# GetOverMassif/QSP-SLAM

Hardware: AMD Instinct MI355X
Metric: joint-opt iters/sec (BA+SDF) (higher is better)
Workload: dtype f32 as 2 x fp16 per operand (hi + 2^-11 lo'), 3 fp16 products per multiply-add, f32 accumulate (decoder); f64 (bundle adjustment)

## Files before the change

include/qsp_hip.h:

```cpp
#ifndef QSP_HIP_H
#define QSP_HIP_H

#include <stddef.h>
#include <stdint.h>

#ifdef __cplusplus
extern "C" {
#endif

enum {
    QSP_OK = 0,
    QSP_ERR_INVALID = 1,
    QSP_ERR_UNSUPPORTED = 2,
    QSP_ERR_DEVICE = 3,
    QSP_ERR_NO_DEVICE = 4
};

const char* qsp_last_error(void);
int qsp_version(void);
int qsp_device_count(void);


typedef struct {
    int32_t n_layers;
    int32_t code_len;
    int32_t latent_in_layer;
    const int32_t* in_dim;
    const int32_t* out_dim;
    const float* const* weight;
    const float* const* weight_g;
    const float* const* bias;
} qsp_decoder_desc;

typedef struct qsp_decoder qsp_decoder;

int qsp_decoder_create(const qsp_decoder_desc* desc, int device, qsp_decoder** out);
void qsp_decoder_destroy(qsp_decoder* dec);

enum { QSP_DEC_OPT_FORWARD_PRECISION = 1, QSP_DEC_OPT_JACOBIAN_PRECISION = 2, QSP_DEC_OPT_TILE_POINTS = 3,
       QSP_DEC_OPT_RENDER_SCREENING = 4, QSP_DEC_OPT_USE_TANH = 5, QSP_DEC_OPT_RANGE_FALLBACK = 6,
       QSP_DEC_OPT_SCREENING_MIN_SAMPLES = 7, QSP_DEC_OPT_NARROW_TILE = 8, QSP_DEC_OPT_SCREEN_AUDIT = 9,
       QSP_DEC_OPT_DEPTH_STAGING = 10 };
enum { QSP_DEC_CNT_RANGE_FALLBACKS = 1, QSP_DEC_CNT_ARENA_REUSED = 2, QSP_DEC_CNT_ARENA_CREATED = 3, QSP_DEC_CNT_NARROW_TILE = 4,
       QSP_DEC_CNT_SCREEN_FALLBACKS = 5 };
int64_t qsp_decoder_get_counter(qsp_decoder* dec, int32_t counter);
int qsp_decoder_set_option(qsp_decoder* dec, int32_t option, int32_t value);

int qsp_decode_sdf(qsp_decoder* dec, const float* code, const float* xyz, int64_t n, float* sdf_out);

int qsp_decode_sdf_screen(qsp_decoder* dec, const float* code, const float* xyz, int64_t n, float* s1_out);

int qsp_sdf_value_grad(qsp_decoder* dec, const float* code, const float* xyz, int64_t n, float* y, float* grad);

typedef struct {
    float k1, k2, k3, k4;
    float b1, b2;
    float lr;
    float s_damp;
    float cut_off;
    int32_t n_iter;
    int32_t n_depth;
    int32_t code_len;
} qsp_joint_cfg;

typedef struct qsp_refine_batch qsp_refine_batch;

int qsp_refine_batch_create(qsp_decoder* dec, const qsp_joint_cfg* cfg, int32_t n_obj,
                            const float* const* pts, const int32_t* n_pts,
                            const float* const* rays, const int32_t* n_rays,
                            const float* const* depth, const int32_t* n_fg,
                            int32_t n_hyp, const int32_t* hyp_obj, qsp_refine_batch** out);
void qsp_refine_batch_destroy(qsp_refine_batch* b);

int qsp_refine_batch_set_state(qsp_refine_batch* b, const float* t_cam_obj, const float* code);

int qsp_refine_batch_run(qsp_refine_batch* b, int32_t n_iter);

int qsp_refine_batch_get(qsp_refine_batch* b, float* t_cam_obj_out, float* code_out, float* loss_out,
                         uint8_t* is_good_out);

int qsp_refine_batch_trace(qsp_refine_batch* b, float* H, float* rhs, float* dx, int32_t* n_valid,
                           int32_t* n_render, float* loss_terms);
int qsp_refine_batch_trace_rot(qsp_refine_batch* b, float* rot4);

int qsp_refine_batch_rows(qsp_refine_batch* b, int enable, int32_t hyp, float* rows_sdf, float* rows_render);

typedef struct {
    float ms_total;
    float ms_mlp_jtj;
    float ms_mlp_fwd;
    float ms_other;
    int32_t n_launch_jtj, n_launch_fwd;
    int64_t pts_jtj;
    int64_t pts_fwd;
    int64_t tiles_jtj, tiles_fwd;
    int64_t pts_band;
    int32_t range_fallbacks;
    int32_t screen_fallbacks;
    float screen_max_diff;
    int32_t screen_audit_failures;
    int64_t pts_audit;
} qsp_refine_profile;
int qsp_refine_batch_profile(qsp_refine_batch* b, int enable, qsp_refine_profile* out);
// ... 490 lines not shown
```

qsp_slam_amd/_lib.py:

```python
import ctypes as C
import os

import numpy as np

_HERE = os.path.dirname(os.path.abspath(__file__))
LIB_PATH = os.environ.get("QSP_HIP_LIB", os.path.join(_HERE, "libqsp_hip.so"))

QSP_OK, QSP_ERR_INVALID, QSP_ERR_UNSUPPORTED, QSP_ERR_DEVICE, QSP_ERR_NO_DEVICE = 0, 1, 2, 3, 4

c_float_p = C.POINTER(C.c_float)
c_double_p = C.POINTER(C.c_double)
c_int32_p = C.POINTER(C.c_int32)
c_int64_p = C.POINTER(C.c_int64)
c_uint8_p = C.POINTER(C.c_uint8)


class QspError(RuntimeError):
    def __init__(self, code, msg):
        RuntimeError.__init__(self, "qsp_hip error %d: %s" % (code, msg))
        self.code = code


class DecoderDesc(C.Structure):
    _fields_ = [("n_layers", C.c_int32), ("code_len", C.c_int32), ("latent_in_layer", C.c_int32),
# ... 137 lines not shown
class FuseOut(C.Structure):
    _fields_ = [("best_idx", c_int32_p), ("best_dist", c_int32_p), ("reason", c_int32_p), ("level", c_int32_p)]


class SearchProjIn(C.Structure):
    _fields_ = [("mode", C.c_int32), ("frame", C.POINTER(OrbFrame)), ("K", C.c_float * 5), ("Ow", C.c_float * 3), ("mb", C.c_float),
                ("u_right", c_float_p), ("slot_blocked", c_uint8_p), ("kp_angle", c_float_p),
                ("th", C.c_float), ("nn_ratio", C.c_float), ("view_cos_limit", C.c_float), ("check_orientation", C.c_int32), ("mono", C.c_int32),
                ("last_Rcw", C.c_float * 9), ("last_tcw", C.c_float * 3), ("n_src", C.c_int32),
                ("src_valid", c_uint8_p), ("src_blocks", c_uint8_p), ("Xw", c_float_p), ("desc", c_uint8_p), ("normal", c_float_p),
                ("dist_min_inv", c_float_p), ("dist_max_inv", c_float_p), ("dist_max", c_float_p), ("src_octave", c_int32_p), ("src_angle", c_float_p)]


class SearchProjOut(C.Structure):
    _fields_ = [("choice", c_int32_p), ("dist", c_int32_p), ("slot_src", c_int32_p), ("in_view", c_uint8_p), ("proj_x", c_float_p),
                ("proj_y", c_float_p), ("proj_xr", c_float_p), ("level", c_int32_p), ("view_cos", c_float_p), ("reason", c_int32_p),
                ("dist2", c_int32_p), ("level_best", c_int32_p), ("level2", c_int32_p), ("bin", c_int32_p), ("n_matches", C.c_int32),
                ("hist", C.c_int32 * 30), ("ind", C.c_int32 * 3), ("n_rounds", C.c_int32)]


class SearchProjKfIn(C.Structure):
    _fields_ = [("mode", C.c_int32), ("frame", C.POINTER(OrbFrame)), ("K", C.c_float * 4), ("Ow", C.c_float * 3),
                ("slot_blocked", c_uint8_p), ("kp_angle", c_float_p), ("th", C.c_float), ("orb_dist", C.c_int32),
                ("check_orientation", C.c_int32), ("n_src", C.c_int32), ("src_valid", c_uint8_p), ("Xw", c_float_p), ("desc", c_uint8_p),
                ("dist_min_inv", c_float_p), ("dist_max_inv", c_float_p), ("dist_max", c_float_p), ("normal", c_float_p),
                ("src_angle", c_float_p)]


class SearchProjKfOut(C.Structure):
    _fields_ = [("choice", c_int32_p), ("dist", c_int32_p), ("slot_src", c_int32_p), ("reason", c_int32_p), ("level", c_int32_p),
                ("proj_x", c_float_p), ("proj_y", c_float_p), ("bin", c_int32_p), ("n_matches", C.c_int32),
                ("hist", C.c_int32 * 30), ("ind", C.c_int32 * 3), ("n_rounds", C.c_int32)]


class TriangulateFrame(C.Structure):
    _fields_ = [("n", C.c_int32), ("Rcw", C.c_float * 9), ("tcw", C.c_float * 3), ("Ow", C.c_float * 3),
                ("fx", C.c_float), ("fy", C.c_float), ("cx", C.c_float), ("cy", C.c_float), ("invfx", C.c_float), ("invfy", C.c_float),
                ("mb", C.c_float), ("mbf", C.c_float), ("xy_un", c_float_p), ("xy", c_float_p), ("u_right", c_float_p), ("depth", c_float_p),
                ("sigma2", c_float_p), ("scale", c_float_p)]


class TriangulateGeom(C.Structure):
    _fields_ = [("n_cand", C.c_int32), ("kf1", C.POINTER(TriangulateFrame)), ("kf2", C.POINTER(TriangulateFrame)), ("ratio_factor", C.c_float)]


class TriangulateOut(C.Structure):
    _fields_ = [("accept", c_uint8_p), ("first", c_uint8_p), ("x3D", c_float_p), ("n_new", c_int32_p), ("reason", c_int32_p), ("path", c_int32_p),
                ("cos_rays", c_float_p), ("z", c_float_p), ("err2", c_float_p), ("ratio_dist", c_float_p)]


SYMBOLS = [
    "qsp_last_error", "qsp_version", "qsp_device_count",
    "qsp_decoder_create", "qsp_decoder_destroy", "qsp_decoder_set_option", "qsp_decoder_get_counter", "qsp_decode_sdf",
    "qsp_decode_sdf_screen", "qsp_sdf_value_grad",
    "qsp_refine_batch_create", "qsp_refine_batch_destroy", "qsp_refine_batch_set_state", "qsp_refine_batch_run",
    "qsp_refine_batch_get", "qsp_refine_batch_trace", "qsp_refine_batch_trace_rot", "qsp_refine_batch_profile", "qsp_refine_batch_rows",
    "qsp_reconstruct_objects", "qsp_estimate_pose", "qsp_refine_detections",
    "qsp_decoder_group_create", "qsp_decoder_group_destroy", "qsp_refine_batch_create_group", "qsp_reconstruct_objects_group",
    "qsp_estimate_pose_group", "qsp_refine_detections_group",
    "qsp_mesh_extractor_create", "qsp_mesh_extractor_destroy", "qsp_mesh_extract", "qsp_mesh_from_volume", "qsp_mesh_fetch", "qsp_mesh_fetch_f64", "qsp_mesh_extractor_set_method",
    "qsp_mesh_extract_batch", "qsp_mesh_from_volumes", "qsp_mesh_fetch_batch", "qsp_mesh_extractor_set_batch_limit",
    "qsp_mesh_extractor_create_group", "qsp_mesh_extract_batch_group",
    "qsp_mc_tables",
    "qsp_pose_optimizer_create", "qsp_pose_optimizer_destroy", "qsp_pose_optimize", "qsp_ellipsoid_fit_planes", "qsp_ellipsoid_fit_prior",
    "qsp_sim3_optimize_batch", "qsp_sim3_ransac_batch", "qsp_search_by_sim3_batch", "qsp_search_by_bow_batch", "qsp_search_for_triangulation_batch", "qsp_fuse_batch", "qsp_search_by_projection", "qsp_search_by_projection_kf", "qsp_triangulate_batch", "qsp_create_new_map_points_batch", "qsp_essential_graph_optimize", "qsp_essential_graph_stages", "qsp_object_gates",
    "qsp_ba_create", "qsp_ba_destroy", "qsp_ba_set_levels", "qsp_ba_optimize", "qsp_ba_local_joint",
    "qsp_ba_set_state", "qsp_ba_get_state", "qsp_ba_get_edges", "qsp_ba_get_index", "qsp_ba_profile", "qsp_ba_set_shard", "qsp_ba_set_deterministic",
    "qsp_ba_set_shard_rccl", "qsp_ba_set_option", "qsp_ba_release_caches", "qsp_comm_unique_id", "qsp_comm_create", "qsp_comm_adopt", "qsp_comm_destroy", "qsp_comm_nccl", "qsp_comm_stub_counts",
    "qsp_comm_rank", "qsp_comm_world", "qsp_comm_allreduce_f64", "qsp_comm_allgather_f32",
]


def lib():
    global _lib
    if _lib is not None:
        return _lib
    if not os.path.isfile(LIB_PATH):
        raise QspError(QSP_ERR_NO_DEVICE, "libqsp_hip.so not built (%s); run qsp_slam_amd/csrc/build.sh -- there is "
                       "no CPU fallback" % LIB_PATH)
    L = C.CDLL(LIB_PATH)
    L.qsp_last_error.restype = C.c_char_p
    L.qsp_version.restype = C.c_int
    L.qsp_device_count.restype = C.c_int
    vp = C.c_void_p
    L.qsp_decoder_create.argtypes = [C.POINTER(DecoderDesc), C.c_int, C.POINTER(vp)]
    L.qsp_decoder_destroy.argtypes = [vp]
    L.qsp_decoder_set_option.argtypes = [vp, C.c_int32, C.c_int32]
    L.qsp_decoder_get_counter.argtypes = [vp, C.c_int32]
    L.qsp_decoder_get_counter.restype = C.c_int64
    L.qsp_decoder_destroy.restype = None
    L.qsp_decode_sdf.argtypes = [vp, c_float_p, c_float_p, C.c_int64, c_float_p]
    L.qsp_decode_sdf_screen.argtypes = [vp, c_float_p, c_float_p, C.c_int64, c_float_p]
    L.qsp_sdf_value_grad.argtypes = [vp, c_float_p, c_float_p, C.c_int64, c_float_p, c_float_p]
    pp_f = C.POINTER(c_float_p)
    L.qsp_refine_batch_create.argtypes = [vp, C.POINTER(JointCfg), C.c_int32, pp_f, c_int32_p, pp_f, c_int32_p, pp_f,
                                          c_int32_p, C.c_int32, c_int32_p, C.POINTER(vp)]
    L.qsp_refine_batch_destroy.argtypes = [vp]
    L.qsp_refine_batch_destroy.restype = None
    L.qsp_refine_batch_set_state.argtypes = [vp, c_float_p, c_float_p]
    L.qsp_refine_batch_run.argtypes = [vp, C.c_int32]
    L.qsp_refine_batch_get.argtypes = [vp, c_float_p, c_float_p, c_float_p, c_uint8_p]
    L.qsp_refine_batch_trace.argtypes = [vp, c_float_p, c_float_p, c_float_p, c_int32_p, c_int32_p, c_float_p]
    L.qsp_refine_batch_trace_rot.argtypes = [vp, c_float_p]
    L.qsp_refine_batch_profile.argtypes = [vp, C.c_int, C.POINTER(RefineProfile)]
    L.qsp_refine_batch_rows.argtypes = [vp, C.c_int, C.c_int32, c_float_p, c_float_p]
    L.qsp_reconstruct_objects.argtypes = [vp, C.POINTER(JointCfg), C.c_int32, pp_f, c_int32_p, pp_f, c_int32_p, pp_f,
                                          c_int32_p, C.c_int32, c_int32_p, c_float_p, c_float_p, c_float_p, c_float_p,
                                          c_float_p, c_uint8_p]
    L.qsp_estimate_pose.argtypes = [vp, C.c_int32, c_float_p, c_float_p, pp_f, c_int32_p, c_float_p, C.c_int32,
                                    c_float_p]
    L.qsp_refine_detections.argtypes = [vp, C.POINTER(JointCfg), C.POINTER(Detections), C.POINTER(DetectionResults)]
    L.qsp_decoder_group_create.argtypes = [C.POINTER(vp), C.c_int32, C.POINTER(vp)]
    L.qsp_decoder_group_destroy.argtypes = [vp]
    L.qsp_decoder_group_destroy.restype = None
    L.qsp_refine_batch_create_group.argtypes = [vp, C.POINTER(JointCfg), C.c_int32, pp_f, c_int32_p, pp_f, c_int32_p, pp_f,
                                                c_int32_p, c_int32_p, C.c_int32, c_int32_p, C.POINTER(vp)]
    L.qsp_reconstruct_objects_group.argtypes = [vp, C.POINTER(JointCfg), C.c_int32, pp_f, c_int32_p, pp_f, c_int32_p, pp_f,
                                                c_int32_p, c_int32_p, C.c_int32, c_int32_p, c_float_p, c_float_p, c_float_p,
                                                c_float_p, c_float_p, c_uint8_p]
    L.qsp_estimate_pose_group.argtypes = [vp, C.c_int32, c_float_p, c_float_p, pp_f, c_int32_p, c_float_p, c_int32_p, C.c_int32,
                                          c_float_p]
    L.qsp_refine_detections_group.argtypes = [vp, C.POINTER(JointCfg), C.POINTER(Detections), c_int32_p, C.POINTER(DetectionResults)]
    L.qsp_mesh_extractor_create.argtypes = [vp, C.c_int32, c_float_p, C.POINTER(vp)]
    L.qsp_mesh_extractor_destroy.argtypes = [vp]
    L.qsp_mesh_extractor_destroy.restype = None
    L.qsp_mesh_extract.argtypes = [vp, c_float_p, c_int64_p, c_int64_p]
    L.qsp_mesh_from_volume.argtypes = [vp, c_float_p, c_int64_p, c_int64_p]
    L.qsp_mesh_fetch.argtypes = [vp, c_float_p, c_int32_p, c_float_p]
    L.qsp_mesh_fetch_f64.argtypes = [vp, C.POINTER(C.c_double)]
    L.qsp_mesh_extractor_set_method.argtypes = [vp, C.c_int32]
    L.qsp_mesh_extract_batch.argtypes = [vp, C.c_int32, c_float_p, c_int64_p, c_int64_p]
    L.qsp_mesh_from_volumes.argtypes = [vp, C.c_int32, c_float_p, c_int64_p, c_int64_p]
    L.qsp_mesh_fetch_batch.argtypes = [vp, c_float_p, C.POINTER(C.c_double), c_int32_p, c_float_p]
    L.qsp_mesh_extractor_set_batch_limit.argtypes = [vp, C.c_int32]
    L.qsp_mesh_extractor_create_group.argtypes = [vp, C.c_int32, c_float_p, C.POINTER(vp)]
    L.qsp_mesh_extract_batch_group.argtypes = [vp, C.c_int32, c_float_p, c_int32_p, c_int64_p, c_int64_p]
    L.qsp_mc_tables.argtypes = [C.POINTER(C.c_int8), C.POINTER(C.c_int8)]
    L.qsp_pose_optimizer_create.argtypes = [C.c_int, C.c_int32, C.POINTER(vp)]
    L.qsp_pose_optimizer_destroy.argtypes = [vp]
    L.qsp_pose_optimizer_destroy.restype = None
    L.qsp_pose_optimize.argtypes = [vp, C.c_int32, c_double_p, c_double_p, c_double_p, c_double_p, c_double_p, c_uint8_p,
                                    c_double_p, c_uint8_p, c_int32_p, C.POINTER(PoseTrace)]
    L.qsp_ellipsoid_fit_planes.argtypes = [C.c_int, C.c_int32, c_double_p, c_int32_p, c_double_p, C.c_int32, C.c_int32,
                                           c_double_p, c_double_p, c_int32_p, c_double_p]
    L.qsp_ellipsoid_fit_prior.argtypes = [C.c_int, C.c_int32, c_double_p, c_int32_p, c_double_p, c_int32_p, c_double_p, c_double_p,
# ... 87 lines not shown
```

qsp_slam_amd/csrc/sdf_mlp.hpp:

```cpp
#pragma once
#include <hip/hip_runtime.h>
#include <stdint.h>

namespace qsp {

typedef float f32x16 __attribute__((ext_vector_type(16)));

#ifndef QSP_EXP_VARIANT
#define QSP_EXP_VARIANT 0
#endif
#if (QSP_EXP_VARIANT & 16)
__device__ unsigned long long qsp_dbg_ts[96];
__device__ unsigned long long qsp_dbg_rt[96];
__device__ int qsp_dbg_n;
#define QSP_TS()                                                                        \
    if (blockIdx.x == 0 && blockIdx.y == 0 && threadIdx.x == 0 && ts_n < 96) {          \
        qsp_dbg_rt[ts_n] = __builtin_amdgcn_s_memrealtime();                            \
        qsp_dbg_ts[ts_n++] = __builtin_readcyclecounter();                              \
        qsp_dbg_n = ts_n;                                                               \
    }
#define QSP_TSK(i)                                                                      \
    if (blockIdx.x == 0 && threadIdx.x == 0 && tsk_first) {                             \
        qsp_dbg_rt[80 + (i)] = __builtin_amdgcn_s_memrealtime();                        \
        qsp_dbg_ts[80 + (i)] = __builtin_readcyclecounter();                            \
    }
#else
#define QSP_TS()
#define QSP_TSK(i)
#endif

constexpr int TILE_P = 64;
constexpr int HID = 512;
constexpr int CODE_LEN = 64;
constexpr int NIN = CODE_LEN + 3;
constexpr int SKIP_COL = HID - NIN;
constexpr int K4 = SKIP_COL + 3;
constexpr int KG4 = K4 / 8;
constexpr int K0_PAD = 96;
constexpr int LDA = HID + 4;
constexpr int LDST = 68;
constexpr int STASH_SHIFT = 1;
static_assert((SKIP_COL - STASH_SHIFT) % 4 == 0 && STASH_SHIFT + NIN <= LDST, "stash row: aligned quads of units 444.., 67 inputs");
constexpr int LDJ = 96;
constexpr int NJ = 72;
constexpr int MLP_THREADS = 512;
constexpr int HT_TILES = 6;

struct MlpParams {
    const float4* wf[8];
    const float4* wb[8];
    const float* bias[8];
    const float* w8;
    float b8;
    const float* w0c;
    const float* w4c;
    const float4* w0x;
    const float4* wf3[8];
    const float4* wb3[8];
    const float4* wfh[8];
    const float4* wbh[8];
    const float4* wbh4s;
    int* range_flag;
    int use_tanh;
    int narrow;
    uint8_t skip[8];
    uint8_t ks_in[8];
    uint8_t ks_out[8];
    uint8_t ncb_in[8];
    uint8_t ncb_out[8];
};

__device__ __forceinline__ float mlp_output(float t, int use_tanh, float& dy) {
    float y = tanhf(t);
    dy = 1.f - y * y;
    if (use_tanh) {
        const float y2 = tanhf(y);
        dy = (1.f - y2 * y2) * dy;
        y = y2;
    }
    return y;
}

struct __attribute__((aligned(16))) MlpSmem {
    float act[TILE_P * LDA];
    float stash[TILE_P * LDST];
    float xin[TILE_P * 4];
    float code[CODE_LEN];
    float c0[HID];
    float c4[HID];
    float y[TILE_P];
    float red[8 * TILE_P];
    float rscale[TILE_P];
    float rres[TILE_P];
    float w8[HID];
    float dy[TILE_P];
};

template <bool AG>
__device__ __forceinline__ f32x16 mfma32t(float a, float b, f32x16 c) {
    if (AG) {
        asm("v_mfma_f32_32x32x2_f32 %0, %1, %2, %0" : "+a"(c) : "v"(a), "v"(b));
        return c;
    }
    return __builtin_amdgcn_mfma_f32_32x32x2f32(a, b, c, 0, 0, 0);
}
template <bool AG>
__device__ __forceinline__ void mfma_acc_settle(f32x16& c0, f32x16& c1, f32x16& c2, f32x16& c3) {
    if (AG) asm volatile("s_nop 15\n\ts_nop 7" : "+a"(c0), "+a"(c1), "+a"(c2), "+a"(c3));
}
template <bool AG>
__device__ __forceinline__ void mfma_acc_settle(f32x16& c0) {
    if (AG) asm volatile("s_nop 15\n\ts_nop 7" : "+a"(c0));
// ... 1314 lines not shown
#pragma unroll
                    for (int q = 0; q < 4; ++q)
                        if (k0 + q < NIN) s.stash[p * LDST + STASH_SHIFT + k0 + q] = sk[r][g][q];
                }
            }
        }
        QSP_BWDH(4, KSH, QSP_WBH(3))
        QSP_BWDH(3, KS4, QSP_WBH(2))
        QSP_BWDH(2, KSH, QSP_WBH(1))
        QSP_BWDH(1, KSH, QSP_WBH(1))
#undef QSP_BWDH
        {
            constexpr int BPT = HID / NT;
            float bnext[7 * BPT];
#pragma unroll
            for (int l = 1; l < 8; ++l)
#pragma unroll
                for (int i = 0; i < BPT; ++i) bnext[BPT * (l - 1) + i] = P.bias[l][tid + i * NT];
            __builtin_amdgcn_sched_barrier(0);
            f32x4 gl[NR][4];
            gemm_side_h2<PF, NR, NW, NARROW>(img, P.wbh[0], wave, lane, gl, NARROW ? (int)P.ks_out[0] : KSH);
            const int c0 = side_c0<NR, NW>(wave);
            __syncthreads();
#pragma unroll
            for (int r = 0; r < NR; ++r) {
                if (r >= side_count<NR, NW>(wave)) break;
                const int p = 32 * side_row<NR, NW>(wave, r) + (lane & 31);
#pragma unroll
                for (int g = 0; g < 4; ++g) {
                    const int k0 = 32 * c0 + 8 * g + 4 * h;
                    if (k0 < NIN) {
                        const float* st = s.stash + p * LDST + STASH_SHIFT + k0;
                        f32x4 v;
#pragma unroll
                        for (int q = 0; q < 4; ++q) v[q] = gl[r][g][q] + (k0 + q < NIN ? st[q] : 0.f);
                        *reinterpret_cast<f32x4*>(s.act + p * LDG + k0) = v;
                    }
                }
            }
            __syncthreads();
#pragma unroll
            for (int l = 1; l < 8; ++l)
#pragma unroll
                for (int i = 0; i < BPT; ++i) bias_sh[(l - 1) * HID + tid + i * NT] = bnext[BPT * (l - 1) + i];
        }
    }
#undef QSP_WH
#undef QSP_WBH
#undef QSP_PIN_ACC
}

constexpr int H1_ROWS = 128;
constexpr int LDH1 = HID + 8;
struct __attribute__((aligned(16))) MlpSmemH1 {
    _Float16 img[H1_ROWS * LDH1 + 64];
    float bias[7 * HID];
    float c0[HID];
    float c4[HID];
    float w8[HID];
    float xin[H1_ROWS * 4];
    float y[H1_ROWS];
    float red[4 * H1_ROWS];
};

template <int PF, int NCB>
struct WRingH1 {
    f32x4 q[PF][NCB];
};
template <int PF, int NCB>
__device__ __forceinline__ void ringh1_prime(WRingH1<PF, NCB>& R, const float4* __restrict__ w_, int cs, int lane) {
    gbytes w = (gbytes)w_;
    const uint32_t voff = 16u * lane;
#pragma unroll
    for (int d = 0; d < PF; ++d)
#pragma unroll
        for (int c = 0; c < NCB; ++c) R.q[d][c] = ldw(w + ((size_t)c * cs + (d * 2) * 64) * 16, voff);
}

template <int KS, int PF, int NCB, int NR>
__device__ __forceinline__ void gemm_h1(const _Float16* __restrict__ img, const float4* __restrict__ w_, int cs,
                                        const float4* __restrict__ nw_, int ncs, WRingH1<PF, NCB>& R, f32x16 (&acc)[NR][NCB], int lane) {
    static_assert(KS % PF == 0 && KS >= 2 * PF && PF % 2 == 0 && NR % NCB == 0, "shape");
    constexpr int RPC = NR / NCB;
    gbytes w = (gbytes)w_;
    gbytes nw = (gbytes)nw_;
    uint32_t voff = 16u * lane;
    int b_idx = (lane & 31) * LDH1 + (lane >> 5) * 8;
    asm volatile("" : "+v"(voff), "+v"(b_idx));
    __builtin_amdgcn_s_waitcnt(0x0F70);
    const _Float16* b_row = img + b_idx;
    f16x8 bh[2][NR];
#pragma unroll
    for (int r = 0; r < NR; ++r) bh[0][r] = *reinterpret_cast<const f16x8*>(b_row + r * 32 * LDH1);
#pragma nounroll
    for (int ks = 0; ks < KS; ks += PF) {
        const bool more = ks + PF < KS;
        gbytes fb = more ? w + (size_t)(ks + PF) * 2 * 64 * 16 : nw;
        const size_t fcs = (size_t)(more ? cs : ncs) * 16;
#pragma unroll
        for (int d = 0; d < PF; ++d) {
            const _Float16* nb = b_row + 16 * (ks + d + 1);
#pragma unroll
            for (int c = 0; c < NCB; ++c) {
                const f16x8 wh = as_f16x8(R.q[d][c]);
#pragma unroll
                for (int r = 0; r < NR; ++r) acc[r][c] = __builtin_amdgcn_mfma_f32_32x32x16_f16(wh, bh[d & 1][r], acc[r][c], 0, 0, 0);
                __builtin_amdgcn_sched_barrier(0);
#pragma unroll
                for (int rr = 0; rr < RPC; ++rr)
                    bh[(d & 1) ^ 1][c * RPC + rr] = *reinterpret_cast<const f16x8*>(nb + (c * RPC + rr) * 32 * LDH1);
                if (c > 0) R.q[d][c - 1] = ldw(fb + (c - 1) * fcs + (size_t)(d * 2) * 64 * 16, voff);
                __builtin_amdgcn_sched_barrier(0);
            }
            R.q[d][NCB - 1] = ldw(fb + (NCB - 1) * fcs + (size_t)(d * 2) * 64 * 16, voff);
            __builtin_amdgcn_sched_barrier(0);
        }
    }
}

__device__ __forceinline__ void h1_store4(_Float16* img, int row, int u0, f32x4 v, float& amax) {
    amax = fmaxf(fmaxf(amax, fabsf(v[0])), fmaxf(fabsf(v[1]), fmaxf(fabsf(v[2]), fabsf(v[3]))));
    asm volatile("" : "+v"(amax));
    f16x4 hi;
#pragma unroll
    for (int q = 0; q < 4; ++q) hi[q] = (_Float16)v[q];
    *reinterpret_cast<f16x4*>(img + row * LDH1 + u0) = hi;
}

template <int PF, int NW = 4>
__device__ __forceinline__ void mlp_tile_h1(MlpSmemH1& s, const MlpParams* __restrict__ Pm, float& amax) {
    constexpr int NR = 4, NCB = 16 / NW;
    int tid = threadIdx.x;
    asm volatile("" : "+v"(tid));
    const int wave = __builtin_amdgcn_readfirstlane(tid >> 6);
    const int lane = tid & 63;
    const int h = lane >> 5;
    int oz;
    asm volatile("s_mov_b32 %0, 0" : "=s"(oz));
    const MlpParams& P = Pm[oz];
    f32x16 acc[NR][NCB];
    _Float16* img = s.img;
    if (tid < H1_ROWS) {
        const f32x4 x = lds4(s.xin + 4 * tid);
        f16x8 hi, z;
#pragma unroll
        for (int j = 0; j < 8; ++j) { hi[j] = (_Float16)0.f; z[j] = (_Float16)0.f; }
#pragma unroll
        for (int j = 0; j < 3; ++j) hi[j] = (_Float16)x[j];
        amax = fmaxf(amax, fmaxf(fabsf(x[0]), fmaxf(fabsf(x[1]), fabsf(x[2]))));
        _Float16* d = img + tid * LDH1;
        *reinterpret_cast<f16x8*>(d) = hi;
        *reinterpret_cast<f16x8*>(d + 8) = z;
    }
    const int cb0 = NCB * wave;
    constexpr int KSH = HID / 16, KS4 = K4 / 16, CS = KSH * 2 * 64, CS4 = KS4 * 2 * 64;
#define QSP_WH(L, KS_) (P.wfh[L] + (size_t)(cb0 * (KS_) * 2) * 64)
    WRingH1<PF, NCB> ring;
    ringh1_prime(ring, QSP_WH(1, KSH), CS, lane);
    __syncthreads();
#define QSP_FWD1(L, BIASPTR, GEMM_STMT)                                                                                  \
    _Pragma("unroll") for (int c_ = 0; c_ < NCB; ++c_) _Pragma("unroll") for (int g_ = 0; g_ < 4; ++g_) {                \
        const f32x4 bv_ = lds4((BIASPTR) + 32 * NCB * wave + 32 * c_ + 8 * g_ + 4 * h);                                  \
        _Pragma("unroll") for (int r_ = 0; r_ < NR; ++r_) _Pragma("unroll") for (int q_ = 0; q_ < 4; ++q_)               \
            acc[r_][c_][4 * g_ + q_] = bv_[q_];                                                                        \
        __builtin_amdgcn_sched_barrier(0);                                                                               \
    }                                                                                                                    \
    GEMM_STMT;                                                                                                           \
     \
     \
    _Pragma("unroll") for (int r_ = 0; r_ < NR; ++r_) _Pragma("unroll") for (int c_ = 0; c_ < NCB; ++c_)                 \
        asm volatile("" : "+a"(acc[r_][c_]));                                                                          \
    __syncthreads();                                                                                                     \
    _Pragma("unroll") for (int c_ = 0; c_ < NCB; ++c_) _Pragma("unroll") for (int g_ = 0; g_ < 4; ++g_) {                \
        const int u0_ = 32 * NCB * wave + 32 * c_ + 8 * g_ + 4 * h;                                                      \
        _Pragma("unroll") for (int r_ = 0; r_ < NR; ++r_) {                                                              \
            f32x4 v_;                                                                                                    \
            _Pragma("unroll") for (int q_ = 0; q_ < 4; ++q_) {                                                           \
                const float x_ = acc[r_][c_][4 * g_ + q_];                                                             \
                v_[q_] = x_ > 0.f ? x_ : 0.f;                                                                            \
            }                                                                                                            \
            h1_store4(img, 32 * r_ + (lane & 31), u0_, v_, amax);                                                        \
        }                                                                                                                \
        __builtin_amdgcn_sched_barrier(0);                                                                               \
    }                                                                                                                    \
    __syncthreads();
#define QSP_GEMM1(L, KS_, NXW, NKS) gemm_h1<KS_, PF, NCB, NR>(img, QSP_WH(L, KS_), (KS_) * 2 * 64, NXW, (NKS) * 2 * 64, ring, acc, lane)
    {
        gbytes w = (gbytes)QSP_WH(0, 1);
        const uint32_t voff = 16u * lane;
        const _Float16* b_row = img + (lane & 31) * LDH1 + (lane >> 5) * 8;
        QSP_FWD1(0, s.c0, {
            f16x8 bh0[NR];
            _Pragma("unroll") for (int r = 0; r < NR; ++r) bh0[r] = *reinterpret_cast<const f16x8*>(b_row + r * 32 * LDH1);
            _Pragma("unroll") for (int c = 0; c < NCB; ++c) {
                const f16x8 wh = as_f16x8(ldw(w + (size_t)(c * 2) * 64 * 16, voff));
                _Pragma("unroll") for (int r = 0; r < NR; ++r)
                    acc[r][c] = __builtin_amdgcn_mfma_f32_32x32x16_f16(wh, bh0[r], acc[r][c], 0, 0, 0);
            }
        })
    }
    QSP_FWD1(1, s.bias + 0 * HID, QSP_GEMM1(1, KSH, QSP_WH(2, KSH), KSH))
    QSP_FWD1(2, s.bias + 1 * HID, QSP_GEMM1(2, KSH, QSP_WH(3, KSH), KSH))
    QSP_FWD1(3, s.bias + 2 * HID, QSP_GEMM1(3, KSH, QSP_WH(4, KS4), KS4))
    if (tid < H1_ROWS) {
#pragma unroll
        for (int ci = 0; ci < 3; ++ci) {
            const float x = s.xin[tid * 4 + ci];
            img[tid * LDH1 + SKIP_COL + ci] = (_Float16)x;
        }
    }
    __syncthreads();
    QSP_FWD1(4, s.c4, QSP_GEMM1(4, KS4, QSP_WH(5, KSH), KSH))
    QSP_FWD1(5, s.bias + 4 * HID, QSP_GEMM1(5, KSH, QSP_WH(6, KSH), KSH))
    QSP_FWD1(6, s.bias + 5 * HID, QSP_GEMM1(6, KSH, QSP_WH(7, KSH), KSH))
    QSP_FWD1(7, s.bias + 6 * HID, QSP_GEMM1(7, KSH, QSP_WH(1, KSH), KSH))
#undef QSP_FWD1
#undef QSP_GEMM1
#undef QSP_WH
    if (NW == 4 || wave < 4) {
        const float* w = s.w8 + 128 * wave;
#pragma unroll
        for (int rr = 0; rr < 2; ++rr) {
            const _Float16* a = img + (lane + 64 * rr) * LDH1 + 128 * wave;
            float pa[4] = {0.f, 0.f, 0.f, 0.f};
#pragma unroll
            for (int g = 0; g < 16; ++g) {
                const f16x8 hi = *reinterpret_cast<const f16x8*>(a + 8 * g);
                const f32x4 w0 = lds4(w + 8 * g), w1 = lds4(w + 8 * g + 4);
#pragma unroll
                for (int j = 0; j < 8; ++j) pa[j & 3] = fmaf((float)hi[j], j < 4 ? w0[j] : w1[j - 4], pa[j & 3]);
            }
            s.red[wave * H1_ROWS + lane + 64 * rr] = (pa[0] + pa[1]) + (pa[2] + pa[3]);
        }
    }
    __syncthreads();
    if (tid < H1_ROWS) {
        float t = P.b8;
#pragma unroll
        for (int q = 0; q < 4; ++q) t += s.red[q * H1_ROWS + tid];
        float dy_;
        s.y[tid] = mlp_output(t, P.use_tanh, dy_);
    }
    __syncthreads();
}

}
```

qsp_slam_amd/csrc/sdf_refine.hip:

```cpp
#include <hip/hip_runtime.h>
#include <math.h>
#include <stdint.h>
#include <stdio.h>
#include <stdlib.h>
#include <string.h>

#include <algorithm>
#include <limits>
#include <string>
#include <mutex>
#include <vector>

#include "../../include/qsp_hip.h"
#include "common.hpp"
#include "sdf_mlp.hpp"

#include "sdf_kernels.hpp"

#ifndef QSP_JTJ_WAVES_DEFAULT
#define QSP_JTJ_WAVES_DEFAULT 8
#endif
#ifndef QSP_SCREEN_WAVES_DEFAULT
#define QSP_SCREEN_WAVES_DEFAULT 4
#endif
// ... 147 lines not shown
    const int in_dim[9] = {NIN, HID, HID, HID, HID, HID, HID, HID, HID};
    const int out_dim[9] = {HID, HID, HID, SKIP_COL, HID, HID, HID, HID, 1};
    auto even4 = [](int v, int cap) { v = std::max(4, (v + 1) & ~1); return std::min(v, cap); };
    double macs = 0, full = 0;
    for (int l = 0; l < 8; ++l) {
        const int in = in_dim[l], out = out_dim[l];
        const int n_hidden = (l == 0) ? 0 : (l == 4 ? SKIP_COL : in);
        int w_out = 0, w_in = 0;
        for (int o = 0; o < out; ++o) {
            bool any = B[l][o] != 0.f;
            for (int k = 0; k < in; ++k)
                if (W[l][(size_t)o * in + k] != 0.f) {
                    any = true;
                    if (k < n_hidden) w_in = std::max(w_in, k + 1);
                }
            if (any) w_out = o + 1;
        }
        const bool skip = src[l] < 0;
        d->P.skip[l] = skip ? 1 : 0;
        const int ks_cap = (l == 4) ? K4 / 16 : HID / 16;
        int ks_in = even4((w_in + 15) / 16, ks_cap);
        if (l == 4 && ks_in >= K4 / 16 - 1) ks_in = K4 / 16;
        d->P.ks_in[l] = (uint8_t)ks_in;
        d->P.ks_out[l] = (uint8_t)even4((w_out + 15) / 16, HID / 16);
        d->P.ncb_in[l] = (uint8_t)std::max(1, (w_in + 31) / 32);
        d->P.ncb_out[l] = (uint8_t)std::max(1, (w_out + 31) / 32);
        full += (double)in * out;
        if (!skip) macs += (double)(l == 0 ? in : 16 * ks_in + (l == 4 ? NIN : 0)) * (32.0 * d->P.ncb_out[l]);
    }
    d->narrow_capable = macs < 0.5 * full;
    d->P.narrow = d->narrow_capable ? 1 : 0;
}

static inline uint16_t bf16_rne(float x) {
    uint32_t u;
    memcpy(&u, &x, 4);
    if ((u & 0x7fffffffu) > 0x7f800000u) return (uint16_t)((u >> 16) | 0x40);
    return (uint16_t)((u + 0x7fffu + ((u >> 16) & 1u)) >> 16);
}
static inline float bf16_f32(uint16_t b) {
    const uint32_t u = (uint32_t)b << 16;
    float x;
    memcpy(&x, &u, 4);
    return x;
}
static inline void bf16_split3(float v, uint16_t& hi, uint16_t& mid, uint16_t& lo) {
    hi = bf16_rne(v);
    const float r1 = v - bf16_f32(hi);
    mid = bf16_rne(r1);
    const float r2 = r1 - bf16_f32(mid);
    lo = bf16_rne(r2);
}

static int pack_weights(qsp_decoder* d, const qsp_decoder_desc* desc) {
    if (desc->n_layers < 1 || desc->n_layers > 64) return qsp_fail(QSP_ERR_UNSUPPORTED, "decoder family: layer count");
    std::vector<std::vector<float>> Wsrc(desc->n_layers);
    for (int l = 0; l < desc->n_layers; ++l) {
        const int in = desc->in_dim[l], out = desc->out_dim[l];
        if (in < 1 || out < 1 || in > 4096 || out > 4096 || !desc->weight[l] || !desc->bias[l])
            return qsp_fail(QSP_ERR_UNSUPPORTED, "decoder family: layer dims");
        Wsrc[l].assign((size_t)out * in, 0.f);
        const float* v = desc->weight[l];
        const float* g = (desc->weight_g && desc->weight_g[l]) ? desc->weight_g[l] : nullptr;
        for (int o = 0; o < out; ++o) {
            float sc = 1.f;
            if (g) {
                float ss = 0.f;
                for (int k = 0; k < in; ++k) ss += v[(size_t)o * in + k] * v[(size_t)o * in + k];
                sc = g[o] / sqrtf(ss);
            }
            for (int k = 0; k < in; ++k) Wsrc[l][(size_t)o * in + k] = v[(size_t)o * in + k] * sc;
        }
        d->mac_per_point += (double)in * out;
    }
    std::vector<std::vector<float>> W, Bias;
    std::vector<int> slot_src;
    {
        const int rc = embed_family(desc, Wsrc, W, Bias, slot_src);
        if (rc) return rc;
    }
    d->code_len = desc->code_len;
    equalize_gains(W, Bias);
    narrow_tables(d, W, Bias, slot_src);
    const int in_dim[9] = {NIN, HID, HID, HID, HID, HID, HID, HID, HID};
    const int out_dim[9] = {HID, HID, HID, SKIP_COL, HID, HID, HID, HID, 1};
    auto upload = [&](const std::vector<float>& h, const void** dst) -> int {
        void* p = nullptr;
        QSP_HIP(hipMalloc(&p, h.size() * sizeof(float) + 16384));
        d->allocs.push_back(p);
        QSP_HIP(hipMemcpy(p, h.data(), h.size() * sizeof(float), hipMemcpyHostToDevice));
        *dst = p;
        return QSP_OK;
    };
    for (int l = 0; l < 8; ++l) {
        const int in = in_dim[l], out = out_dim[l];
        int rc = QSP_OK;
        if (l == 0) {
            std::vector<float> wc((size_t)HID * CODE_LEN), wx((size_t)(HID / 4) * 3 * 4);
            for (int o = 0; o < HID; ++o)
                for (int k = 0; k < CODE_LEN; ++k) wc[(size_t)k * HID + o] = W[0][(size_t)o * in + k];
            for (int q = 0; q < HID / 4; ++q)
                for (int a = 0; a < 3; ++a)
                    for (int e = 0; e < 4; ++e) wx[((size_t)q * 3 + a) * 4 + e] = W[0][(size_t)(4 * q + e) * in + CODE_LEN + a];
            rc = upload(wc, (const void**)&d->P.w0c);
            if (!rc) rc = upload(wx, (const void**)&d->P.w0x);
            d->P.wf[0] = nullptr;
            d->P.wf3[0] = nullptr;
            if (!rc) {
                std::vector<_Float16> ph((size_t)16 * 2 * 64 * 8, (_Float16)0.f);
                for (int cb = 0; cb < 16; ++cb)
                    for (int lane = 0; lane < 64; ++lane)
                        for (int j = 0; j < 8; ++j) {
                            const int o = 32 * cb + (lane & 31), k = 8 * (lane >> 5) + j;
                            float v = 0.f;
                            if (o < out && k < 3) v = W[0][(size_t)o * in + CODE_LEN + k];
                            if (!(fabsf(v) < 65000.f)) d->fp16_ok = false;
                            const _Float16 hi = (_Float16)v;
                            const size_t base = ((size_t)cb * 2) * 64 * 8 + (size_t)lane * 8 + j;
                            ph[base] = hi;
                            ph[base + 64 * 8] = (_Float16)((v - (float)hi) * 2048.f);
                        }
                void* phd = nullptr;
                QSP_HIP(hipMalloc(&phd, ph.size() * sizeof(_Float16) + 16384));
                d->allocs.push_back(phd);
                QSP_HIP(hipMemcpy(phd, ph.data(), ph.size() * sizeof(_Float16), hipMemcpyHostToDevice));
                d->P.wfh[0] = (const float4*)phd;
            }
        } else {
            const int KG = (l == 4) ? KG4 : HID / 8;
            std::vector<float> pf((size_t)16 * KG * 64 * 4, 0.f);
            for (int cb = 0; cb < 16; ++cb)
                for (int kg = 0; kg < KG; ++kg)
                    for (int lane = 0; lane < 64; ++lane)
                        for (int e = 0; e < 4; ++e) {
                            const int o = 32 * cb + (lane & 31);
                            int k = 8 * kg + 4 * (lane >> 5) + e;
                            if (l == 4 && k >= SKIP_COL) k += CODE_LEN;
                            float v = 0.f;
                            if (o < out && k < in) v = W[l][(size_t)o * in + k];
                            pf[(((size_t)cb * KG + kg) * 64 + lane) * 4 + e] = v;
                        }
            rc = upload(pf, (const void**)&d->P.wf[l]);
            if (!rc) {
                const int KS = KG / 2;
                std::vector<uint16_t> p3((size_t)16 * KS * 3 * 64 * 8, 0);
                for (int cb = 0; cb < 16; ++cb)
                    for (int ks = 0; ks < KS; ++ks)
                        for (int lane = 0; lane < 64; ++lane)
                            for (int j = 0; j < 8; ++j) {
                                const int o = 32 * cb + (lane & 31);
                                int k = 16 * ks + 8 * (lane >> 5) + j;
                                if (l == 4 && k >= SKIP_COL) k += CODE_LEN;
                                float v = 0.f;
                                if (o < out && k < in) v = W[l][(size_t)o * in + k];
                                uint16_t hi, mid, lo;
                                bf16_split3(v, hi, mid, lo);
                                const size_t base = (((size_t)cb * KS + ks) * 3) * 64 * 8 + (size_t)lane * 8 + j;
                                p3[base] = hi;
                                p3[base + 64 * 8] = mid;
                                p3[base + 2 * 64 * 8] = lo;
                            }
                void* p3d = nullptr;
                QSP_HIP(hipMalloc(&p3d, p3.size() * sizeof(uint16_t) + 16384));
                d->allocs.push_back(p3d);
                QSP_HIP(hipMemcpy(p3d, p3.data(), p3.size() * sizeof(uint16_t), hipMemcpyHostToDevice));
                d->P.wf3[l] = (const float4*)p3d;
            }
            if (!rc) {
                const int KS = KG / 2;
                std::vector<_Float16> ph((size_t)16 * KS * 2 * 64 * 8, (_Float16)0.f);
                for (int cb = 0; cb < 16; ++cb)
                    for (int ks = 0; ks < KS; ++ks)
                        for (int lane = 0; lane < 64; ++lane)
                            for (int j = 0; j < 8; ++j) {
                                const int o = 32 * cb + (lane & 31);
                                int k = 16 * ks + 8 * (lane >> 5) + j;
                                if (l == 4 && k >= SKIP_COL) k += CODE_LEN;
                                float v = 0.f;
                                if (o < out && k < in) v = W[l][(size_t)o * in + k];
                                if (!(fabsf(v) < 65000.f)) d->fp16_ok = false;
                                const _Float16 hi = (_Float16)v;
                                const _Float16 lo = (_Float16)((v - (float)hi) * 2048.f);
                                const size_t base = (((size_t)cb * KS + ks) * 2) * 64 * 8 + (size_t)lane * 8 + j;
                                ph[base] = hi;
                                ph[base + 64 * 8] = lo;
                            }
                void* phd = nullptr;
                QSP_HIP(hipMalloc(&phd, ph.size() * sizeof(_Float16) + 16384));
                d->allocs.push_back(phd);
                QSP_HIP(hipMemcpy(phd, ph.data(), ph.size() * sizeof(_Float16), hipMemcpyHostToDevice));
                d->P.wfh[l] = (const float4*)phd;
            }
            if (!rc && l == 4) {
                std::vector<float> wc((size_t)HID * CODE_LEN);
                for (int o = 0; o < HID; ++o)
                    for (int k = 0; k < CODE_LEN; ++k) wc[(size_t)k * HID + o] = W[4][(size_t)o * in + SKIP_COL + k];
                rc = upload(wc, (const void**)&d->P.w4c);
            }
        }
        if (rc) return rc;
        const int NCB = (l == 0) ? 3 : 16;
        const int OG = HID / 8;
        std::vector<float> pb((size_t)NCB * OG * 64 * 4, 0.f);
        for (int cb = 0; cb < NCB; ++cb)
            for (int og = 0; og < OG; ++og)
                for (int lane = 0; lane < 64; ++lane)
                    for (int e = 0; e < 4; ++e) {
                        const int k = 32 * cb + (lane & 31);
                        const int o = 8 * og + 4 * (lane >> 5) + e;
                        float v = 0.f;
                        if (o < out && k < in) v = W[l][(size_t)o * in + k];
                        pb[(((size_t)cb * OG + og) * 64 + lane) * 4 + e] = v;
                    }
        rc = upload(pb, (const void**)&d->P.wb[l]);
        if (rc) return rc;
        {
            const int KS = HID / 16;
            std::vector<uint16_t> p3((size_t)NCB * KS * 3 * 64 * 8, 0);
            for (int cb = 0; cb < NCB; ++cb)
                for (int ks = 0; ks < KS; ++ks)
                    for (int lane = 0; lane < 64; ++lane)
                        for (int j = 0; j < 8; ++j) {
                            const int k = 32 * cb + (lane & 31);
                            const int o = 16 * ks + 8 * (lane >> 5) + j;
                            float v = 0.f;
                            if (o < out && k < in) v = W[l][(size_t)o * in + k];
                            uint16_t hi, mid, lo;
                            bf16_split3(v, hi, mid, lo);
                            const size_t base = (((size_t)cb * KS + ks) * 3) * 64 * 8 + (size_t)lane * 8 + j;
                            p3[base] = hi;
                            p3[base + 64 * 8] = mid;
                            p3[base + 2 * 64 * 8] = lo;
                        }
            void* p3d = nullptr;
            QSP_HIP(hipMalloc(&p3d, p3.size() * sizeof(uint16_t) + 16384));
            d->allocs.push_back(p3d);
            QSP_HIP(hipMemcpy(p3d, p3.data(), p3.size() * sizeof(uint16_t), hipMemcpyHostToDevice));
            d->P.wb3[l] = (const float4*)p3d;
        }
        {
            const int KS = HID / 16;
            std::vector<_Float16> ph((size_t)NCB * KS * 2 * 64 * 8, (_Float16)0.f);
            for (int cb = 0; cb < NCB; ++cb)
                for (int ks = 0; ks < KS; ++ks)
// ... 1308 lines not shown
```

Baseline: 5633.

## Switch screening MLP GEMMs to 16x16x32 MFMA with repacked fp16 weights

Templates the hi-only (screening) MLP tile on MFMA shape and makes the 16x16x32 f16 instruction the default instead of 32x32x16. It adds a new weight packing (wh16) laid out for the 16-wide tiles, uploads it per layer, and exposes a packing entry point. The smaller tile shape changes accumulator register use, the LDS access pattern and the bias/epilogue indexing. The cost is an extra weight copy in device memory and different instruction scheduling.

Result: no change. 5650, median of 6 (+0.3%).

```diff
diff --git a/include/qsp_hip.h b/include/qsp_hip.h
--- a/include/qsp_hip.h
+++ b/include/qsp_hip.h
@@ -49,6 +49,8 @@
 int qsp_decode_sdf(qsp_decoder* dec, const float* code, const float* xyz, int64_t n, float* sdf_out);
 
 int qsp_decode_sdf_screen(qsp_decoder* dec, const float* code, const float* xyz, int64_t n, float* s1_out);
+
+int64_t qsp_pack_screen_weights(int32_t layer, const float* W, int32_t out_dim, int32_t in_dim, uint16_t* planes, int64_t cap);
 
 int qsp_sdf_value_grad(qsp_decoder* dec, const float* code, const float* xyz, int64_t n, float* y, float* grad);
 
diff --git a/qsp_slam_amd/_lib.py b/qsp_slam_amd/_lib.py
--- a/qsp_slam_amd/_lib.py
+++ b/qsp_slam_amd/_lib.py
@@ -213,7 +213,7 @@
 SYMBOLS = [
     "qsp_last_error", "qsp_version", "qsp_device_count",
     "qsp_decoder_create", "qsp_decoder_destroy", "qsp_decoder_set_option", "qsp_decoder_get_counter", "qsp_decode_sdf",
-    "qsp_decode_sdf_screen", "qsp_sdf_value_grad",
+    "qsp_decode_sdf_screen", "qsp_pack_screen_weights", "qsp_sdf_value_grad",
     "qsp_refine_batch_create", "qsp_refine_batch_destroy", "qsp_refine_batch_set_state", "qsp_refine_batch_run",
     "qsp_refine_batch_get", "qsp_refine_batch_trace", "qsp_refine_batch_trace_rot", "qsp_refine_batch_profile", "qsp_refine_batch_rows",
     "qsp_reconstruct_objects", "qsp_estimate_pose", "qsp_refine_detections",
@@ -252,6 +252,8 @@
     L.qsp_decoder_destroy.restype = None
     L.qsp_decode_sdf.argtypes = [vp, c_float_p, c_float_p, C.c_int64, c_float_p]
     L.qsp_decode_sdf_screen.argtypes = [vp, c_float_p, c_float_p, C.c_int64, c_float_p]
+    L.qsp_pack_screen_weights.argtypes = [C.c_int32, c_float_p, C.c_int32, C.c_int32, C.POINTER(C.c_uint16), C.c_int64]
+    L.qsp_pack_screen_weights.restype = C.c_int64
     L.qsp_sdf_value_grad.argtypes = [vp, c_float_p, c_float_p, C.c_int64, c_float_p, c_float_p]
     pp_f = C.POINTER(c_float_p)
     L.qsp_refine_batch_create.argtypes = [vp, C.POINTER(JointCfg), C.c_int32, pp_f, c_int32_p, pp_f, c_int32_p, pp_f,
diff --git a/qsp_slam_amd/csrc/sdf_mlp.hpp b/qsp_slam_amd/csrc/sdf_mlp.hpp
--- a/qsp_slam_amd/csrc/sdf_mlp.hpp
+++ b/qsp_slam_amd/csrc/sdf_mlp.hpp
@@ -58,6 +58,7 @@
     const float4* wf3[8];
     const float4* wb3[8];
     const float4* wfh[8];
+    const float4* wh16[8];
     const float4* wbh[8];
     const float4* wbh4s;
     int* range_flag;
@@ -1478,6 +1479,10 @@
 
 constexpr int H1_ROWS = 128;
 constexpr int LDH1 = HID + 8;
+#ifndef QSP_H1_SHAPE
+#define QSP_H1_SHAPE 16
+#endif
+constexpr int H1_SHAPE = QSP_H1_SHAPE;
 struct __attribute__((aligned(16))) MlpSmemH1 {
     _Float16 img[H1_ROWS * LDH1 + 64];
     float bias[7 * HID];
@@ -1489,56 +1494,74 @@
     float red[4 * H1_ROWS];
 };
 
+template <int SHAPE> struct H1Shape;
+template <> struct H1Shape<32> {
+    static constexpr int T = 32, SK = 16, PL = 2;
+    typedef f32x16 acc_t;
+    static __device__ __forceinline__ const float4* weights(const MlpParams& P, int l) { return P.wfh[l]; }
+    static __device__ __forceinline__ acc_t mfma(f16x8 a, f16x8 b, acc_t c) { return __builtin_amdgcn_mfma_f32_32x32x16_f16(a, b, c, 0, 0, 0); }
+};
+template <> struct H1Shape<16> {
+    static constexpr int T = 16, SK = 32, PL = 1;
+    typedef f32x4 acc_t;
+    static __device__ __forceinline__ const float4* weights(const MlpParams& P, int l) { return P.wh16[l]; }
+    static __device__ __forceinline__ acc_t mfma(f16x8 a, f16x8 b, acc_t c) { return __builtin_amdgcn_mfma_f32_16x16x32_f16(a, b, c, 0, 0, 0); }
+};
+
 template <int PF, int NCB>
 struct WRingH1 {
     f32x4 q[PF][NCB];
 };
-template <int PF, int NCB>
+template <int SHAPE, int PF, int NCB>
 __device__ __forceinline__ void ringh1_prime(WRingH1<PF, NCB>& R, const float4* __restrict__ w_, int cs, int lane) {
+    constexpr int PL = H1Shape<SHAPE>::PL;
     gbytes w = (gbytes)w_;
     const uint32_t voff = 16u * lane;
 #pragma unroll
     for (int d = 0; d < PF; ++d)
 #pragma unroll
-        for (int c = 0; c < NCB; ++c) R.q[d][c] = ldw(w + ((size_t)c * cs + (d * 2) * 64) * 16, voff);
-}
-
-template <int KS, int PF, int NCB, int NR>
+        for (int c = 0; c < NCB; ++c) R.q[d][c] = ldw(w + ((size_t)c * cs + (d * PL) * 64) * 16, voff);
+}
+
+template <int SHAPE, int KS, int PF, int NCB, int NR>
 __device__ __forceinline__ void gemm_h1(const _Float16* __restrict__ img, const float4* __restrict__ w_, int cs,
-                                        const float4* __restrict__ nw_, int ncs, WRingH1<PF, NCB>& R, f32x16 (&acc)[NR][NCB], int lane) {
+                                        const float4* __restrict__ nw_, int ncs, WRingH1<PF, NCB>& R,
+                                        typename H1Shape<SHAPE>::acc_t (&acc)[NR][NCB], int lane) {
+    typedef H1Shape<SHAPE> SH;
+    constexpr int T = SH::T, SK = SH::SK, PL = SH::PL;
     static_assert(KS % PF == 0 && KS >= 2 * PF && PF % 2 == 0 && NR % NCB == 0, "shape");
     constexpr int RPC = NR / NCB;
     gbytes w = (gbytes)w_;
     gbytes nw = (gbytes)nw_;
     uint32_t voff = 16u * lane;
-    int b_idx = (lane & 31) * LDH1 + (lane >> 5) * 8;
+    int b_idx = (lane & (T - 1)) * LDH1 + (lane / T) * 8;
     asm volatile("" : "+v"(voff), "+v"(b_idx));
     __builtin_amdgcn_s_waitcnt(0x0F70);
     const _Float16* b_row = img + b_idx;
     f16x8 bh[2][NR];
 #pragma unroll
-    for (int r = 0; r < NR; ++r) bh[0][r] = *reinterpret_cast<const f16x8*>(b_row + r * 32 * LDH1);
+    for (int r = 0; r < NR; ++r) bh[0][r] = *reinterpret_cast<const f16x8*>(b_row + r * T * LDH1);
 #pragma nounroll
     for (int ks = 0; ks < KS; ks += PF) {
         const bool more = ks + PF < KS;
-        gbytes fb = more ? w + (size_t)(ks + PF) * 2 * 64 * 16 : nw;
+        gbytes fb = more ? w + (size_t)(ks + PF) * PL * 64 * 16 : nw;
         const size_t fcs = (size_t)(more ? cs : ncs) * 16;
 #pragma unroll
         for (int d = 0; d < PF; ++d) {
-            const _Float16* nb = b_row + 16 * (ks + d + 1);
+            const _Float16* nb = b_row + SK * (ks + d + 1);
 #pragma unroll
             for (int c = 0; c < NCB; ++c) {
                 const f16x8 wh = as_f16x8(R.q[d][c]);
 #pragma unroll
-                for (int r = 0; r < NR; ++r) acc[r][c] = __builtin_amdgcn_mfma_f32_32x32x16_f16(wh, bh[d & 1][r], acc[r][c], 0, 0, 0);
+                for (int r = 0; r < NR; ++r) acc[r][c] = SH::mfma(wh, bh[d & 1][r], acc[r][c]);
                 __builtin_amdgcn_sched_barrier(0);
 #pragma unroll
                 for (int rr = 0; rr < RPC; ++rr)
-                    bh[(d & 1) ^ 1][c * RPC + rr] = *reinterpret_cast<const f16x8*>(nb + (c * RPC + rr) * 32 * LDH1);
-                if (c > 0) R.q[d][c - 1] = ldw(fb + (c - 1) * fcs + (size_t)(d * 2) * 64 * 16, voff);
+                    bh[(d & 1) ^ 1][c * RPC + rr] = *reinterpret_cast<const f16x8*>(nb + (c * RPC + rr) * T * LDH1);
+                if (c > 0) R.q[d][c - 1] = ldw(fb + (c - 1) * fcs + (size_t)(d * PL) * 64 * 16, voff);
                 __builtin_amdgcn_sched_barrier(0);
             }
-            R.q[d][NCB - 1] = ldw(fb + (NCB - 1) * fcs + (size_t)(d * 2) * 64 * 16, voff);
+            R.q[d][NCB - 1] = ldw(fb + (NCB - 1) * fcs + (size_t)(d * PL) * 64 * 16, voff);
             __builtin_amdgcn_sched_barrier(0);
         }
     }
@@ -1553,18 +1576,22 @@
     *reinterpret_cast<f16x4*>(img + row * LDH1 + u0) = hi;
 }
 
-template <int PF, int NW = 4>
+template <int PF, int NW = 4, int SHAPE = H1_SHAPE>
 __device__ __forceinline__ void mlp_tile_h1(MlpSmemH1& s, const MlpParams* __restrict__ Pm, float& amax) {
-    constexpr int NR = 4, NCB = 16 / NW;
+    typedef H1Shape<SHAPE> SH;
+    constexpr int T = SH::T, SK = SH::SK, PL = SH::PL;
+    constexpr int NR = H1_ROWS / T, NCB = HID / NW / T;
+    constexpr int NQ = T * T / 256;
+    constexpr int UQ = T / NQ;
     int tid = threadIdx.x;
     asm volatile("" : "+v"(tid));
     const int wave = __builtin_amdgcn_readfirstlane(tid >> 6);
     const int lane = tid & 63;
-    const int h = lane >> 5;
+    const int h = lane / T;
     int oz;
     asm volatile("s_mov_b32 %0, 0" : "=s"(oz));
     const MlpParams& P = Pm[oz];
-    f32x16 acc[NR][NCB];
+    typename SH::acc_t acc[NR][NCB];
     _Float16* img = s.img;
     if (tid < H1_ROWS) {
         const f32x4 x = lds4(s.xin + 4 * tid);
@@ -1576,17 +1603,19 @@
         amax = fmaxf(amax, fmaxf(fabsf(x[0]), fmaxf(fabsf(x[1]), fabsf(x[2]))));
         _Float16* d = img + tid * LDH1;
         *reinterpret_cast<f16x8*>(d) = hi;
-        *reinterpret_cast<f16x8*>(d + 8) = z;
+#pragma unroll
+        for (int j = 8; j < SK; j += 8) *reinterpret_cast<f16x8*>(d + j) = z;
     }
     const int cb0 = NCB * wave;
-    constexpr int KSH = HID / 16, KS4 = K4 / 16, CS = KSH * 2 * 64, CS4 = KS4 * 2 * 64;
-#define QSP_WH(L, KS_) (P.wfh[L] + (size_t)(cb0 * (KS_) * 2) * 64)
+    static_assert(HID % SK == 0 && K4 % SK == 0, "whole slabs");
+    constexpr int KSH = HID / SK, KS4 = K4 / SK, CS = KSH * PL * 64;
+#define QSP_WH(L, KS_) (SH::weights(P, L) + (size_t)(cb0 * (KS_) * PL) * 64)
     WRingH1<PF, NCB> ring;
-    ringh1_prime(ring, QSP_WH(1, KSH), CS, lane);
+    ringh1_prime<SHAPE>(ring, QSP_WH(1, KSH), CS, lane);
     __syncthreads();
 #define QSP_FWD1(L, BIASPTR, GEMM_STMT)                                                                                  \
-    _Pragma("unroll") for (int c_ = 0; c_ < NCB; ++c_) _Pragma("unroll") for (int g_ = 0; g_ < 4; ++g_) {                \
-        const f32x4 bv_ = lds4((BIASPTR) + 32 * NCB * wave + 32 * c_ + 8 * g_ + 4 * h);                                  \
+    _Pragma("unroll") for (int c_ = 0; c_ < NCB; ++c_) _Pragma("unroll") for (int g_ = 0; g_ < NQ; ++g_) {               \
+        const f32x4 bv_ = lds4((BIASPTR) + T * NCB * wave + T * c_ + UQ * g_ + 4 * h);                                   \
         _Pragma("unroll") for (int r_ = 0; r_ < NR; ++r_) _Pragma("unroll") for (int q_ = 0; q_ < 4; ++q_)               \
             acc[r_][c_][4 * g_ + q_] = bv_[q_];                                                                        \
         __builtin_amdgcn_sched_barrier(0);                                                                               \
@@ -1597,31 +1626,31 @@
     _Pragma("unroll") for (int r_ = 0; r_ < NR; ++r_) _Pragma("unroll") for (int c_ = 0; c_ < NCB; ++c_)                 \
         asm volatile("" : "+a"(acc[r_][c_]));                                                                          \
     __syncthreads();                                                                                                     \
-    _Pragma("unroll") for (int c_ = 0; c_ < NCB; ++c_) _Pragma("unroll") for (int g_ = 0; g_ < 4; ++g_) {                \
-        const int u0_ = 32 * NCB * wave + 32 * c_ + 8 * g_ + 4 * h;                                                      \
+    _Pragma("unroll") for (int c_ = 0; c_ < NCB; ++c_) _Pragma("unroll") for (int g_ = 0; g_ < NQ; ++g_) {               \
+        const int u0_ = T * NCB * wave + T * c_ + UQ * g_ + 4 * h;                                                       \
         _Pragma("unroll") for (int r_ = 0; r_ < NR; ++r_) {                                                              \
             f32x4 v_;                                                                                                    \
             _Pragma("unroll") for (int q_ = 0; q_ < 4; ++q_) {                                                           \
                 const float x_ = acc[r_][c_][4 * g_ + q_];                                                             \
                 v_[q_] = x_ > 0.f ? x_ : 0.f;                                                                            \
             }                                                                                                            \
-            h1_store4(img, 32 * r_ + (lane & 31), u0_, v_, amax);                                                        \
+            h1_store4(img, T * r_ + (lane & (T - 1)), u0_, v_, amax);                                                    \
         }                                                                                                                \
         __builtin_amdgcn_sched_barrier(0);                                                                               \
     }                                                                                                                    \
     __syncthreads();
-#define QSP_GEMM1(L, KS_, NXW, NKS) gemm_h1<KS_, PF, NCB, NR>(img, QSP_WH(L, KS_), (KS_) * 2 * 64, NXW, (NKS) * 2 * 64, ring, acc, lane)
+#define QSP_GEMM1(L, KS_, NXW, NKS) \
+    gemm_h1<SHAPE, KS_, PF, NCB, NR>(img, QSP_WH(L, KS_), (KS_) * PL * 64, NXW, (NKS) * PL * 64, ring, acc, lane)
     {
         gbytes w = (gbytes)QSP_WH(0, 1);
         const uint32_t voff = 16u * lane;
-        const _Float16* b_row = img + (lane & 31) * LDH1 + (lane >> 5) * 8;
+        const _Float16* b_row = img + (lane & (T - 1)) * LDH1 + h * 8;
         QSP_FWD1(0, s.c0, {
             f16x8 bh0[NR];
-            _Pragma("unroll") for (int r = 0; r < NR; ++r) bh0[r] = *reinterpret_cast<const f16x8*>(b_row + r * 32 * LDH1);
+            _Pragma("unroll") for (int r = 0; r < NR; ++r) bh0[r] = *reinterpret_cast<const f16x8*>(b_row + r * T * LDH1);
             _Pragma("unroll") for (int c = 0; c < NCB; ++c) {
-                const f16x8 wh = as_f16x8(ldw(w + (size_t)(c * 2) * 64 * 16, voff));
-                _Pragma("unroll") for (int r = 0; r < NR; ++r)
-                    acc[r][c] = __builtin_amdgcn_mfma_f32_32x32x16_f16(wh, bh0[r], acc[r][c], 0, 0, 0);
+                const f16x8 wh = as_f16x8(ldw(w + (size_t)(c * PL) * 64 * 16, voff));
+                _Pragma("unroll") for (int r = 0; r < NR; ++r) acc[r][c] = SH::mfma(wh, bh0[r], acc[r][c]);
             }
         })
     }
diff --git a/qsp_slam_amd/csrc/sdf_refine.hip b/qsp_slam_amd/csrc/sdf_refine.hip
--- a/qsp_slam_amd/csrc/sdf_refine.hip
+++ b/qsp_slam_amd/csrc/sdf_refine.hip
@@ -223,6 +223,41 @@
     lo = bf16_rne(r2);
 }
 
+static int hi16_slabs(int l) { return l == 0 ? 1 : (l == 4 ? K4 : HID) / 32; }
+static bool pack_hi16(int l, const float* W, int out, int in, _Float16* dst) {
+    const int KS = hi16_slabs(l);
+    bool ok = true;
+    for (int cb = 0; cb < HID / 16; ++cb)
+        for (int ks = 0; ks < KS; ++ks)
+            for (int lane = 0; lane < 64; ++lane)
+                for (int j = 0; j < 8; ++j) {
+                    const int o = 16 * cb + (lane & 15);
+                    int k = 32 * ks + 8 * (lane >> 4) + j;
+                    if (l == 0) k = k < 3 ? CODE_LEN + k : in;
+                    else if (l == 4 && k >= SKIP_COL) k += CODE_LEN;
+                    float v = 0.f;
+                    if (o < out && k < in) v = W[(size_t)o * in + k];
+                    if (!(fabsf(v) < 65000.f)) ok = false;
+                    dst[(((size_t)cb * KS + ks) * 64 + lane) * 8 + j] = (_Float16)v;
+                }
+    return ok;
+}
+extern "C" int64_t qsp_pack_screen_weights(int32_t layer, const float* W, int32_t out_dim, int32_t in_dim, uint16_t* planes, int64_t cap) {
+    const int in_want = layer == 0 ? NIN : HID;
+    if (layer < 0 || layer > 7 || !W || out_dim < 1 || out_dim > HID || in_dim != in_want) {
+        qsp_fail(QSP_ERR_INVALID, "qsp_pack_screen_weights: bad argument");
+        return -1;
+    }
+    const int64_t n = (int64_t)(HID / 16) * hi16_slabs(layer) * 64 * 8;
+    if (!planes || cap < n) return n;
+    static_assert(sizeof(_Float16) == sizeof(uint16_t), "fp16 bits");
+    if (!pack_hi16(layer, W, out_dim, in_dim, reinterpret_cast<_Float16*>(planes))) {
+        qsp_fail(QSP_ERR_UNSUPPORTED, "split fp16: a weight of this decoder is outside fp16's range");
+        return -1;
+    }
+    return n;
+}
+
 static int pack_weights(qsp_decoder* d, const qsp_decoder_desc* desc) {
     if (desc->n_layers < 1 || desc->n_layers > 64) return qsp_fail(QSP_ERR_UNSUPPORTED, "decoder family: layer count");
     std::vector<std::vector<float>> Wsrc(desc->n_layers);
@@ -261,6 +296,16 @@
         d->allocs.push_back(p);
         QSP_HIP(hipMemcpy(p, h.data(), h.size() * sizeof(float), hipMemcpyHostToDevice));
         *dst = p;
+        return QSP_OK;
+    };
+    auto upload_hi16 = [&](int l) -> int {
+        std::vector<_Float16> ph((size_t)(HID / 16) * hi16_slabs(l) * 64 * 8);
+        if (!pack_hi16(l, W[l].data(), out_dim[l], in_dim[l], ph.data())) d->fp16_ok = false;
+        void* phd = nullptr;
+        QSP_HIP(hipMalloc(&phd, ph.size() * sizeof(_Float16) + 16384));
+        d->allocs.push_back(phd);
+        QSP_HIP(hipMemcpy(phd, ph.data(), ph.size() * sizeof(_Float16), hipMemcpyHostToDevice));
+        d->P.wh16[l] = (const float4*)phd;
         return QSP_OK;
     };
     for (int l = 0; l < 8; ++l) {
@@ -296,6 +341,7 @@
                 d->allocs.push_back(phd);
                 QSP_HIP(hipMemcpy(phd, ph.data(), ph.size() * sizeof(_Float16), hipMemcpyHostToDevice));
                 d->P.wfh[0] = (const float4*)phd;
+                rc = upload_hi16(0);
             }
         } else {
             const int KG = (l == 4) ? KG4 : HID / 8;
@@ -361,6 +407,7 @@
                 d->allocs.push_back(phd);
                 QSP_HIP(hipMemcpy(phd, ph.data(), ph.size() * sizeof(_Float16), hipMemcpyHostToDevice));
                 d->P.wfh[l] = (const float4*)phd;
+                rc = upload_hi16(l);
             }
             if (!rc && l == 4) {
                 std::vector<float> wc((size_t)HID * CODE_LEN);
```
